# itz-sayak/C-Users-Sayakdutta-Self-Supervised-Arbitrary-Scale-Point-Cloud-Upsampling-via-SNN

Measured on AMD Instinct MI355X. Metric: upsampled query-points/sec (kNN + fn fwd + rotate + fd fwd + displace), 4x scale, M=48 T=4, higher is better.
Workload: dtype f32 (GEMMs as 3 x f16 MFMA with f32 accumulation; outer kNN f64); 1 GPU; synthetic sphere N=5000 (seed 0), B=4096 grid queries per GPU per step, M=48, T=4, fn k=[24,18,12] emb 640, fd k=32 scales [8,16,32,48] emb 768, conditioned-random weights seed 0, in-patch kNN recomputed every batch; cloud_points=5000, neighbours=48, outer_knn=f64 brute force, parallelism=query shards x1

## Files before the change

### c-users-sayakdutta-self-supervised-arbitrary-scale-point-cloud-upsampling-via-snn_amd/_lib.py

```python
import ctypes
import os
from ctypes import POINTER, c_char_p, c_double, c_float, c_int, c_int32, c_int64, c_void_p

_HERE = os.path.dirname(os.path.abspath(__file__))
LIB_PATH = os.environ.get("SAPCU_LIB_PATH") or os.path.join(_HERE, "csrc", "libsapcu_hip.so")
EXACT_LIB_PATH = os.path.join(_HERE, "csrc", "libsapcu_hip_exact.so")

FN_TAPS = ("stem", "block1", "block2", "block3", "pooled", "enc", "logits")
FD_TAPS = ("fused0", "spikes", "knn", "pooled", "enc", "x0")
KIND_FN, KIND_FD = 0, 1
ABI_VERSION = 2


class SapcuLibraryError(RuntimeError):
    """The HIP library is absent or unloadable (never silently replaced by a CPU path)."""


class SapcuError(RuntimeError):
    """A C entry point returned a non-zero status: args = (code, text)."""


_SIGNATURES = {
    "sapcu_abi_version": (c_int, []),
    "sapcu_last_error": (c_char_p, []),
# ... 43 lines not shown
    "sapcu_gemm_f32": (c_int, [c_void_p, c_int64, c_int, c_int, c_void_p, c_int, c_void_p, c_void_p, c_int, c_void_p,
                               c_int, c_void_p, c_int, c_int, c_void_p]),
    "sapcu_to_split_rows": (c_int, [c_void_p, c_int64, c_int, c_int, c_void_p, c_int, c_void_p]),
    "sapcu_posenc_gemm_f32": (c_int, [c_void_p, c_int64, c_int, c_void_p, c_void_p, c_void_p, c_int, c_void_p, c_void_p,
                                      c_int, c_int, c_void_p, c_void_p, c_void_p, c_void_p, c_int, c_void_p]),
    "sapcu_model_gemm_mode": (c_int, [c_void_p, POINTER(c_int), POINTER(c_int)]),
    "sapcu_model_fused_blocks": (c_int, [c_void_p, c_int, POINTER(c_int)]),
    "sapcu_fn_edge_chain_workspace_bytes": (c_int64, [c_int64, c_int, c_int]),
    "sapcu_fn_edge_chain_f32": (c_int, [c_void_p, c_void_p, c_int64, c_int, c_int, c_int] + [c_void_p] * 12 + [c_int, c_int, c_void_p, c_void_p,
                                        c_int64, c_void_p]),
}

EXPORTS = tuple(_SIGNATURES)

_SEEDS_SIGNATURES = {
    "sapcu_dense_seeds_workspace_bytes": (c_int64, [c_int64, c_int64]),
    "sapcu_dense_seeds_f64": (c_int, [c_void_p, c_int64, c_double, c_void_p, c_int64, c_int64, POINTER(c_int64), POINTER(c_int64),
                              c_void_p, c_int64, c_void_p]),
}
SEEDS_EXPORTS = tuple(_SEEDS_SIGNATURES)

_INTERNAL_SIGNATURES = {
    "sapcu_internal_fold_affine_host": (c_int, [c_void_p, c_void_p, c_void_p, c_void_p, c_int, c_int, c_void_p, c_void_p]),
}
_lib = None


def load(path=None):
    global _lib
    if _lib is not None and path is None:
        return _lib
    p = path or LIB_PATH
    if not os.path.exists(p):
        raise SapcuLibraryError(
            "HIP library not built: %s is missing. Run `make -C %s` (needs hipcc, gfx950). "
            "There is no CPU fallback." % (p, os.path.dirname(p)))
    try:
        lib = ctypes.CDLL(p)
    except OSError as e:
        raise SapcuLibraryError("cannot load %s: %s" % (p, e)) from e
    for name, (res, args) in list(_SIGNATURES.items()) + list(_SEEDS_SIGNATURES.items()) + list(_INTERNAL_SIGNATURES.items()):
        try:
            fn = getattr(lib, name)
        except AttributeError as e:
            raise SapcuLibraryError("%s does not export %s" % (p, name)) from e
        fn.restype = res
# ... 22 lines not shown
```

### c-users-sayakdutta-self-supervised-arbitrary-scale-point-cloud-upsampling-via-snn_amd/csrc/fd_encoder.hip

```cpp
#include <type_traits>

#include "common.h"
#include "gemm_epi.h"
#include "ops.h"

namespace sapcu {
typedef _Float16 half8 __attribute__((ext_vector_type(8)));

#ifdef FE_STAMPS
#define FE_STAMP(IDX)                                                                                                   \
    do {                                                                                                                \
        if (a.tap_spikes && threadIdx.x == 0)                                                                           \
            reinterpret_cast<unsigned long long*>(a.tap_spikes)[(int64_t)blockIdx.x * 32 + (IDX)] = __builtin_amdgcn_s_memtime(); \
    } while (0)
#else
#define FE_STAMP(IDX) do { } while (0)
#endif

constexpr int FE_M = 48;
constexpr int FE_NT = 512;
constexpr int FE_XLD = 448;
constexpr int FE_OFF_R2 = 0;
constexpr int FE_R2_BYTES = 65536;
constexpr int FE_OFF_XS = FE_R2_BYTES;
constexpr int FE_OFF_XYZ = FE_OFF_XS + FE_M * FE_XLD * 4;
constexpr int FE_OFF_IDX0 = FE_OFF_XYZ + FE_M * 16;
constexpr int FE_OFF_IDXL = FE_OFF_IDX0 + FE_M * FE_M;
constexpr int FE_OFF_XX = FE_OFF_IDXL + FE_M * FE_M;
constexpr int FE_LDS = 163840;
constexpr int FE_OFF_X3L = FE_OFF_R2 + 32768;
constexpr int FE_OFF_BEST = FE_OFF_XYZ;
static_assert(FE_OFF_BEST + 6 * 4 * 8 * 16 * 4 <= FE_LDS && FE_OFF_X3L + 16 * 512 * 4 <= FE_OFF_XYZ, "fd encoder: multi_scale_conv areas");
constexpr int FE_F_LD = 36;
constexpr int FE_KEYS_OFF = 2 * 64 * FE_F_LD * 4;
constexpr int FE_TLD = 36;
constexpr int FE_TILE = FE_M * FE_TLD;
static_assert(8 * FE_TILE * 4 <= FE_R2_BYTES, "fd encoder: staging tiles");
static_assert(FE_OFF_XX + 256 <= FE_LDS && FE_LDS <= 163840, "fd encoder: LDS budget");
static_assert(FE_KEYS_OFF + FE_M * (FE_M + 1) * 4 <= FE_R2_BYTES, "fd encoder: score keys");
// ... 107 lines not shown
#pragma unroll
                for (int i = 0; i < RC; ++i)
#pragma unroll
                    for (int j = hc * HC; j < (hc + 1) * HC && j < NCS; ++j)
                        acc[rc * RC + i][j] = __builtin_amdgcn_mfma_f32_16x16x32_f16(ah[i], wh[j], acc[rc * RC + i][j], 0, 0, 0);
            }
            __builtin_amdgcn_sched_barrier(0);
#pragma unroll
            for (int j = hc * HC; j < (hc + 1) * HC && j < NCS; ++j) {
                wh[j] = fe_wfrag(wp, nk_all, cs[j], sn, 0, lane);
                wl[j] = fe_wfrag(wp, nk_all, cs[j], sn, 1, lane);
            }
        }
    }
    if (Wh) {
#pragma unroll
        for (int j = 0; j < NCARRY; ++j) {
            (*Wh)[j] = wh[j];
            (*Wl)[j] = wl[j];
        }
    }
}

__device__ __forceinline__ int fe_wave_sum(int v) {
    v += __builtin_amdgcn_update_dpp(0, v, 0xB1, 0xF, 0xF, true);
    v += __builtin_amdgcn_update_dpp(0, v, 0x4E, 0xF, 0xF, true);
    v += __builtin_amdgcn_update_dpp(0, v, 0x141, 0xF, 0xF, true);
    v += __builtin_amdgcn_update_dpp(0, v, 0x140, 0xF, 0xF, true);
    return __builtin_amdgcn_readlane(v, 0) + __builtin_amdgcn_readlane(v, 16) + __builtin_amdgcn_readlane(v, 32) +
           __builtin_amdgcn_readlane(v, 48);
}

template <typename Fill>
__device__ __forceinline__ void fe_knn(unsigned char* R2, float* xx, unsigned char* idx_out, int m, int c, int k, Fill fill,
                                       int32_t* __restrict__ tap, int tid) {
    float* Fb = reinterpret_cast<float*>(R2);
    unsigned* K = reinterpret_cast<unsigned*>(R2 + FE_KEYS_OFF);
    const int lane = tid & 63, wave = __builtin_amdgcn_readfirstlane(tid >> 6);
    const int r16 = lane & 15, g4 = lane >> 4;
    const int bi0 = 0, bj0 = wave < 3 ? wave : 0;
    const int bi1 = wave == 1 ? 2 : 1, bj1 = wave == 2 ? 1 : 2;
    f32x4 acc0 = {0.f, 0.f, 0.f, 0.f}, acc1 = {0.f, 0.f, 0.f, 0.f};
    float myxx = 0.f;
    __syncthreads();
    if (wave >= 4) fill(Fb, 0, min(32, c), tid - 256);
    __syncthreads();
    int buf = 0;
    for (int c0 = 0; c0 < c; c0 += 32, buf ^= 1) {
        const int cw = min(32, c - c0);
        const float* F = Fb + buf * (64 * FE_F_LD);
        if (wave >= 4) {
            if (c0 + 32 < c) fill(Fb + (buf ^ 1) * (64 * FE_F_LD), c0 + 32, min(32, c - c0 - 32), tid - 256);
        } else if (wave < 3) {
            const float* fa0 = F + (16 * bi0 + r16) * FE_F_LD + g4;
            const float* fb0 = F + (16 * bj0 + r16) * FE_F_LD + g4;
            const float* fa1 = F + (16 * bi1 + r16) * FE_F_LD + g4;
            const float* fb1 = F + (16 * bj1 + r16) * FE_F_LD + g4;
            if (cw == 32) {
// ... 7 lines not shown
                }
#pragma unroll
                for (int s4 = 0; s4 < 8; ++s4) {
                    acc0 = __builtin_amdgcn_mfma_f32_16x16x4f32(a0[s4], b0[s4], acc0, 0, 0, 0);
                    acc1 = __builtin_amdgcn_mfma_f32_16x16x4f32(a1[s4], b1[s4], acc1, 0, 0, 0);
                }
            } else {
                for (int cc = 0; cc < cw; cc += 4) {
                    acc0 = __builtin_amdgcn_mfma_f32_16x16x4f32(fa0[cc], fb0[cc], acc0, 0, 0, 0);
                    acc1 = __builtin_amdgcn_mfma_f32_16x16x4f32(fa1[cc], fb1[cc], acc1, 0, 0, 0);
                }
            }
        } else if (lane < m) {
            const float* fr = F + lane * FE_F_LD;
            for (int cc2 = 0; cc2 < cw; ++cc2) {
                const float sq = __fmul_rn(fr[cc2], fr[cc2]);
                myxx = (c0 == 0 && cc2 == 0) ? sq : __fadd_rn(myxx, sq);
            }
        }
        __syncthreads();
    }
    if (wave == 3 && lane < m) xx[lane] = myxx;
    __syncthreads();
    if (wave < 3) {
#pragma unroll
        for (int q = 0; q < 2; ++q) {
            const int bi = q ? bi1 : bi0, bj = q ? bj1 : bj0;
            const f32x4 acc = q ? acc1 : acc0;
            const int j = 16 * bj + r16;
#pragma unroll
            for (int e = 0; e < 4; ++e) {
                const int i = 16 * bi + 4 * g4 + e;
                if (i < m && j < m) {
                    const float inner = __fmul_rn(-2.0f, acc[e]);
                    K[i * (m + 1) + j] = float_max_key(__fadd_rn(__fsub_rn(__fsub_rn(-xx[j], inner), xx[i]), 0.0f));
                    if (bi != bj) K[j * (m + 1) + i] = float_max_key(__fadd_rn(__fsub_rn(__fsub_rn(-xx[i], inner), xx[j]), 0.0f));
                }
            }
        }
    }
    __syncthreads();
    const int full = m * (m - 1) / 2;
    for (int i = wave; i < m; i += FE_NT / 64) {
        const unsigned key0 = lane < m ? K[i * (m + 1) + lane] : 0u;
        int r0 = 0;
        for (int jb = 0; jb < m; jb += 8) {
#pragma unroll
            for (int u = 0; u < 8; ++u) r0 += (unsigned)__builtin_amdgcn_readlane(key0, (jb + u) & 63) > key0;
        }
        const int tot = fe_wave_sum(lane < m ? r0 : 0);
        if (tot != full) {
            const unsigned long long k0 = ((unsigned long long)key0 << 32) | (unsigned)~lane;
            r0 = 0;
            for (int jb = 0; jb < m; jb += 8) {
#pragma unroll
                for (int u = 0; u < 8; ++u) {
                    const int jp = jb + u;
                    const unsigned long long kv = ((unsigned long long)(unsigned)__builtin_amdgcn_readlane(key0, jp & 63) << 32) | (unsigned)~jp;
                    r0 += kv > k0;
                }
            }
        }
        if (lane < m && r0 < k) {
            idx_out[i * FE_M + r0] = (unsigned char)lane;
            if (tap) tap[i * k + r0] = lane;
        }
    }
}

constexpr int FE_PR = 64;
constexpr int FE_TP = FE_M / 3;

__device__ __forceinline__ void fe_put_at(unsigned char* p, float v) {
    v = settle(v);
    const _Float16 hi = (_Float16)v;
    *reinterpret_cast<_Float16*>(p) = hi;
    *reinterpret_cast<_Float16*>(p + FE_PR * 64) = (_Float16)__builtin_fmaf((float)hi, -1.0f, v);
}

template <int KIND, bool FAST>
__device__ __forceinline__ void fe_emit4(const float (&x)[4], const NeuronP& p, int t0, int nemit, unsigned char* const (&pe)[4], int pt0,
                                         int m, bool count, int* __restrict__ gate, float* __restrict__ tap, int64_t tap_tstride) {
    const int total = FAST ? 4 : t0 + nemit;
    {
        NeuronStep2<KIND == 1> n0(p), n1(p);
        const f32x2 z = f32x2{0.f, 0.f};
        bool o0 = false, o1 = false;
        if (FAST) {
// ... 70 lines not shown
            if (a.tap_knn) a.tap_knn[tab_off + e] = v;
        }
    } else {
        FeNP pn = fe_load_np(a.nprm, COFF_IN + (tid & 31));
        auto fill = [&](float* F, int c0, int cw, int ftid) {
            const int cc = ftid & 31;
            const NeuronP p = fe_np(pn);
            pn = fe_load_np(a.nprm, COFF_IN + (c0 + 32 < CIN ? c0 + 32 : c0) + cc);
#pragma unroll
            for (int n = 0; n < 8; n += 2) {
                const int ia = (ftid >> 5) + 8 * n, ib = ia + 8;
                if (ia < FE_M) {
                    const f32x2 sp = fe_spike0<KIND_IN>(f32x2{XS[ia * FE_XLD + COFF_IN + c0 + cc],
                                                              XS[(ib < FE_M ? ib : ia) * FE_XLD + COFF_IN + c0 + cc]}, p);
                    F[ia * FE_F_LD + cc] = ia < m ? sp.x : 0.f;
                    F[ib * FE_F_LD + cc] = (ib < m && ib < FE_M) ? sp.y : 0.f;
                } else {
                    F[ia * FE_F_LD + cc] = 0.f;
                    F[ib * FE_F_LD + cc] = 0.f;
                }
            }
            (void)cw;
        };
        fe_knn(R2, xx, IDXL, m, CIN, kk, fill, a.tap_knn ? a.tap_knn + tab_off : nullptr, tid);
    }
    __syncthreads();
    FE_STAMP(4 * L);
    {
        const int cc = tid & 63;
        FeNP pn2 = fe_load_np(a.nprm, COFF_IN + cc);
        for (int c0 = 0; c0 < CIN; c0 += 64) {
            const NeuronP p = fe_np(pn2);
            pn2 = fe_load_np(a.nprm, COFF_IN + (c0 + 64 < CIN ? c0 + 64 : c0) + cc);
#pragma unroll
            for (int n = 0; n < 6; n += 2) {
                const int ia = (tid >> 6) + 8 * n, ib = ia + 8;
                const f32x2 sp = fe_spike0<KIND_IN>(f32x2{XS[ia * FE_XLD + COFF_IN + c0 + cc], XS[ib * FE_XLD + COFF_IN + c0 + cc]}, p);
                fe_put<64>(R2, ia, c0 + cc, sp.x);
                fe_put<64>(R2, ib, c0 + cc, sp.y);
#ifdef FE_DEBUG_PANEL
                if (a.tap_x0 && ia < m) a.tap_x0[((a.s0 + patch_i) * m + ia) * 960 + COFF_IN + c0 + cc] = sp.x;
                if (a.tap_x0 && ib < m) a.tap_x0[((a.s0 + patch_i) * m + ib) * 960 + COFF_IN + c0 + cc] = sp.y;
#endif
            }
        }
    }
    __syncthreads();
    FE_STAMP(4 * L + 1);
    const bool active = L != 1 || w < 4;
    f32x4 acc[NPW][3][4];
    if (active) {
#pragma unroll
        for (int q = 0; q < NPW; ++q) {
            const int pr = w + 8 * q;
            const int css[4] = {2 * pr, 2 * pr + 1, 2 * (COUT / 32 + pr), 2 * (COUT / 32 + pr) + 1};
            fe_gemm16<4, 3>(R2, 4096, reinterpret_cast<const half8*>(a.edge_wp[L - 1]), CIN / 32, css, lane, acc[q]);
        }
    }
    __syncthreads();
    FE_STAMP(4 * L + 2);
    float* SAw = reinterpret_cast<float*>(R2) + w * FE_TILE;
    const int c16 = lane & 15, g4 = lane >> 4;
    const int qd = lane & 7, g6 = 6 * (lane >> 3);
#pragma unroll
    for (int q = 0; q < NPW; ++q) {
        float pre[3][2][4];
        if (active) {
            const int col0 = 32 * (w + 8 * q) + c16;
            const float sh[2] = {a.shift[L - 1][col0], a.shift[L - 1][col0 + 16]};
#pragma unroll
            for (int rs = 0; rs < 3; ++rs)
#pragma unroll
                for (int cj = 0; cj < 2; ++cj)
#pragma unroll
                    for (int e = 0; e < 4; ++e)
                        SAw[(16 * rs + 4 * g4 + e) * FE_TLD + 16 * cj + c16] = __fadd_rn(__fmul_rn(acc[q][rs][cj][e], 0.0625f), 0.0f);
            asm volatile("s_waitcnt lgkmcnt(0)" ::: "memory");
            __builtin_amdgcn_wave_barrier();
            {
                float4 mx[6];
#pragma unroll
                for (int r = 0; r < 6; ++r) mx[r] = make_float4(-__builtin_huge_valf(), -__builtin_huge_valf(), -__builtin_huge_valf(), -__builtin_huge_valf());
                const unsigned char* ir0 = IDXL + g6 * FE_M;
                const float* tq = SAw + 4 * qd;
                int j = 0;
                for (; j + 4 <= kk; j += 4) {
                    unsigned pk[6];
#pragma unroll
                    for (int r = 0; r < 6; ++r) pk[r] = *reinterpret_cast<const unsigned*>(ir0 + r * FE_M + j);
#pragma unroll
                    for (int r = 0; r < 6; ++r) {
                        const float4 v0 = *reinterpret_cast<const float4*>(tq + (pk[r] & 255u) * FE_TLD);
                        const float4 v1 = *reinterpret_cast<const float4*>(tq + ((pk[r] >> 8) & 255u) * FE_TLD);
                        const float4 v2 = *reinterpret_cast<const float4*>(tq + ((pk[r] >> 16) & 255u) * FE_TLD);
                        const float4 v3 = *reinterpret_cast<const float4*>(tq + (pk[r] >> 24) * FE_TLD);
                        mx[r].x = fmaxf(fmaxf(mx[r].x, v0.x), fmaxf(v1.x, fmaxf(v2.x, v3.x)));
                        mx[r].y = fmaxf(fmaxf(mx[r].y, v0.y), fmaxf(v1.y, fmaxf(v2.y, v3.y)));
                        mx[r].z = fmaxf(fmaxf(mx[r].z, v0.z), fmaxf(v1.z, fmaxf(v2.z, v3.z)));
                        mx[r].w = fmaxf(fmaxf(mx[r].w, v0.w), fmaxf(v1.w, fmaxf(v2.w, v3.w)));
                    }
                }
                for (; j < kk; ++j) {
#pragma unroll
                    for (int r = 0; r < 6; ++r) {
                        const float4 v0 = *reinterpret_cast<const float4*>(tq + ir0[r * FE_M + j] * FE_TLD);
                        mx[r].x = fmaxf(mx[r].x, v0.x);
                        mx[r].y = fmaxf(mx[r].y, v0.y);
                        mx[r].z = fmaxf(mx[r].z, v0.z);
                        mx[r].w = fmaxf(mx[r].w, v0.w);
                    }
                }
                asm volatile("s_waitcnt lgkmcnt(0)" ::: "memory");
                __builtin_amdgcn_wave_barrier();
#pragma unroll
                for (int r = 0; r < 6; ++r) *reinterpret_cast<float4*>(SAw + (g6 + r) * FE_TLD + 4 * qd) = mx[r];
                asm volatile("s_waitcnt lgkmcnt(0)" ::: "memory");
                __builtin_amdgcn_wave_barrier();
            }
#pragma unroll
            for (int rs = 0; rs < 3; ++rs)
#pragma unroll
                for (int cj = 0; cj < 2; ++cj)
#pragma unroll
                    for (int e = 0; e < 4; ++e) {
                        const int row = 16 * rs + 4 * g4 + e;
                        const float mxv = SAw[row * FE_TLD + 16 * cj + c16];
                        const float xb = __fadd_rn(__fmul_rn(acc[q][rs][2 + cj][e], 0.0625f), 0.0f);
                        pre[rs][cj][e] = lrelu02(__fadd_rn(__fsub_rn(mxv, xb), sh[cj]));
                        if (a.tap_x0 && row < m) a.tap_x0[((a.s0 + patch_i) * m + row) * 960 + COFF_OUT + col0 + 16 * cj] = pre[rs][cj][e];
                    }
            asm volatile("s_waitcnt lgkmcnt(0)" ::: "memory");
            __builtin_amdgcn_wave_barrier();
            if (L <= 2) {
#pragma unroll
                for (int rs = 0; rs < 3; ++rs)
#pragma unroll
                    for (int cj = 0; cj < 2; ++cj)
#pragma unroll
                        for (int e = 0; e < 4; ++e) XS[(16 * rs + 4 * g4 + e) * FE_XLD + COFF_OUT + col0 + 16 * cj] = pre[rs][cj][e];
            } else {
#pragma unroll
                for (int rs = 0; rs < 3; ++rs)
#pragma unroll
                    for (int cj = 0; cj < 2; ++cj)
#pragma unroll
                        for (int e = 0; e < 4; ++e) SAw[(16 * rs + 4 * g4 + e) * FE_TLD + 16 * cj + c16] = pre[rs][cj][e];
            }
        }
        if (L == 3) {
            __syncthreads();
            const float* SA = reinterpret_cast<const float*>(R2);
#pragma unroll
            for (int jj = 0; jj < 2; ++jj) {
                const int c3l = 2 * jj + 1 - (w & 1);
#pragma unroll
                for (int th = 0; th < 3; ++th)
#pragma unroll
                    for (int e = 0; e < 4; ++e)
                        x3[th][2 * q + jj][e] = SA[(2 * c3l + (lane >> 5)) * FE_TILE + (FE_TP * th + 4 * (w >> 1) + e) * FE_TLD + (lane & 31)];
            }
            __syncthreads();
        }
    }
    __syncthreads();
    FE_STAMP(4 * L + 3);
}

template <bool GENERAL>
__global__ __launch_bounds__(FE_NT, 1) void fd_encoder_kernel(const FdEncArgs a) {
    extern __shared__ __attribute__((aligned(1024))) unsigned char smem[];
    float* XS = reinterpret_cast<float*>(smem + FE_OFF_XS);
    unsigned char* R2 = smem + FE_OFF_R2;
    float4* XYZ = reinterpret_cast<float4*>(smem + FE_OFF_XYZ);
    unsigned char* IDX0 = smem + FE_OFF_IDX0;
    float* xx = reinterpret_cast<float*>(smem + FE_OFF_XX);
    const int tid = threadIdx.x;
    const int lane = tid & 63, w = __builtin_amdgcn_readfirstlane(tid >> 6);
    const int m = a.m;
    const int64_t patch_i = blockIdx.x;
    const float* __restrict__ pp = a.patch + patch_i * m * 3;

    for (int e = tid; e < FE_M; e += FE_NT)
        XYZ[e] = e < m ? make_float4(pp[3 * e], pp[3 * e + 1], pp[3 * e + 2], 0.f) : make_float4(0.f, 0.f, 0.f, 0.f);
    for (int e = tid; e < 2 * FE_M * FE_M / 4; e += FE_NT) reinterpret_cast<unsigned*>(IDX0)[e] = 0u;
    __syncthreads();
    FE_STAMP(0);
    {
        auto fill = [&](float* F, int c0, int cw, int ftid) {
            {
                const int i = ftid >> 2, cc = ftid & 3;
                const float v = reinterpret_cast<const float*>(XYZ)[4 * (i < FE_M ? i : 0) + cc];
                F[i * FE_F_LD + cc] = i < m ? v : 0.f;
            }
            (void)c0; (void)cw;
        };
        fe_knn(R2, xx, IDX0, m, 3, a.kmax0, fill, nullptr, tid);
    }
    __syncthreads();
    FE_STAMP(1);
    {
        const float* XYZf = reinterpret_cast<const float*>(XYZ);
        const int r16 = lane & 15, g4 = lane >> 4;
        float wb[4][4][2], bb[4];
#pragma unroll
        for (int sc = 0; sc < 4; ++sc) {
#pragma unroll
            for (int ct = 0; ct < 4; ++ct)
#pragma unroll
                for (int kstep = 0; kstep < 2; ++kstep) {
                    const int k = 4 * kstep + g4;
                    wb[sc][ct][kstep] = (sc < a.nscale && k < 6) ? a.e0_w[((int64_t)sc * 64 + 16 * ct + r16) * 6 + k] : 0.f;
                }
            bb[sc] = sc < a.nscale ? a.e0_b[sc * 64 + lane] : 0.f;
        }
        int ksv[4];
#pragma unroll
        for (int sc = 0; sc < 4; ++sc) ksv[sc] = sc < a.nscale ? a.ks[sc] : 0;
        float big = 0.f;
        for (int i = w; i < m; i += FE_NT / 64) {
// ... 174 lines not shown
                FE_TACC(fe_t_epi);
            };
            third(std::integral_constant<int, 0>{});
            third(std::integral_constant<int, 1>{});
            third(std::integral_constant<int, 2>{});
            if (cbw < ncb) {
                int lane_e = lane;
                asm volatile("" : "+v"(lane_e));
                const float* bl = BESTL;
                asm volatile("" : "+v"(bl));
                const int tt = lane_e >> 4, r16e = lane_e & 15;
#pragma unroll
                for (int j = 0; j < 6; ++j) {
                    const float bias = a.msc_b[16 * css[j] + r16e];
                    const float raw = bl[512 * j];
                    if (tt < nemit)
                        a.pooled[((int64_t)(t0 + tt) * a.b + patch_i) * a.emb + 16 * css[j] + r16e] = lrelu02(__fadd_rn(__fmul_rn(raw, 0.0625f), bias));
                }
            }
        }
    }
#ifdef FE_STAMPS
    if (a.tap_spikes && threadIdx.x == 0) {
        unsigned long long* st = reinterpret_cast<unsigned long long*>(a.tap_spikes) + (int64_t)blockIdx.x * 32;
        st[17] = fe_t_emit;
        st[18] = fe_t_mfma;
        st[28] = fe_t_start;
        st[29] = fe_t_epi;
        st[19] = __builtin_amdgcn_s_memtime();
    }
#endif
}

constexpr int FM_OFF_BEST = 32768;
constexpr int FM_LDS = FM_OFF_BEST + 6 * 4 * 8 * 16 * 4;

template <bool GENERAL>
__global__ __launch_bounds__(FE_NT, 1) void fd_msc_kernel(const FdMscArgs a) {
    extern __shared__ __attribute__((aligned(1024))) unsigned char smem[];
    unsigned char* R2 = smem;
    const int tid = threadIdx.x;
    const int lane = tid & 63, w = __builtin_amdgcn_readfirstlane(tid >> 6);
    const int m = a.m;
    const int64_t patch_i = blockIdx.x;
    const float* __restrict__ xp = a.x0 + patch_i * m * 960;
    const int cw = w & 1, rg = w >> 1;
    const int nsweep = a.emb / 768 + (a.emb % 768 ? 1 : 0);
// ... 178 lines not shown
```

### c-users-sayakdutta-self-supervised-arbitrary-scale-point-cloud-upsampling-via-snn_amd/csrc/model.hip

```cpp
#include <stdarg.h>
#include <stdlib.h>

#include <new>
#include <vector>

#include "common.h"
#include "ops.h"

namespace sapcu {

static thread_local char g_err[512] = "";

void set_error(const char* fmt, ...) {
    va_list ap;
    va_start(ap, fmt);
    vsnprintf(g_err, sizeof(g_err), fmt, ap);
    va_end(ap);
}

enum FnSlot {
    FN_STEM_W = 0, FN_STEM_B, FN_STEM_LIF,
    FN_BLK0 = 3,
    FN_FINAL_W = FN_BLK0 + 63, FN_FINAL_B, FN_FINAL_LIF,
    FN_FCOUT_W, FN_FCOUT_B,
// ... 976 lines not shown
        if (m->w16_hi) (void)hipFree(m->w16_hi);
        if (m->w16_lo) (void)hipFree(m->w16_lo);
        if (m->chain_w) (void)hipFree(m->chain_w);
        if (m->ovf_dev) (void)hipFree(m->ovf_dev);
        if (m->blob) (void)hipFree(m->blob);
        if (m->ks_dev) (void)hipFree(m->ks_dev);
        if (m->gate_dev) (void)hipFree(m->gate_dev);
        if (m->fde_w) (void)hipFree(m->fde_w);
        if (m->fde_nprm) (void)hipFree(m->fde_nprm);
        delete m;
        return rc;
    }
    *out = m;
    return SAPCU_OK;
}

int sapcu_internal_fold_affine_host(const float* w_out, const float* b_out, const float* w_fc2, const float* b_fc2, int d, int n,
                                    float* w_fold_out, float* b_fold_out) {
    SAPCU_CHECK_ARG(w_out && b_out && w_fc2 && b_fc2 && w_fold_out && b_fold_out && d >= 1 && n >= 1, "fold_affine: bad argument");
    fold_affine_f64(w_out, b_out, w_fc2, b_fc2, d, n, w_fold_out, b_fold_out);
    return SAPCU_OK;
}

int sapcu_model_destroy(sapcu_model_t m) {
    if (!m) return SAPCU_OK;
    if (m->w16_hi) (void)hipFree(m->w16_hi);
    if (m->w16_lo) (void)hipFree(m->w16_lo);
    if (m->chain_w) (void)hipFree(m->chain_w);
    if (m->ovf_dev) (void)hipFree(m->ovf_dev);
    if (m->blob) (void)hipFree(m->blob);
    if (m->ks_dev) (void)hipFree(m->ks_dev);
    if (m->gate_dev) (void)hipFree(m->gate_dev);
    if (m->fde_w) (void)hipFree(m->fde_w);
    if (m->fde_nprm) (void)hipFree(m->fde_nprm);
    delete m;
    return SAPCU_OK;
}

int64_t sapcu_workspace_bytes(sapcu_model_t m, int64_t b, int m_pts) {
    if (!m || b < 0 || m_pts < 1 || m_pts > 128) {
        set_error("workspace_bytes: bad argument");
        return SAPCU_ERR_ARG;
    }
    return m->kind == SAPCU_KIND_FN ? fn_ws_bytes(m, b, m_pts) : fd_ws_bytes(m, b, m_pts);
}

// ... 48 lines not shown
```

### c-users-sayakdutta-self-supervised-arbitrary-scale-point-cloud-upsampling-via-snn_amd/csrc/ops.h

```cpp
#pragma once
#include "common.h"

namespace sapcu {

int launch_patch_knn_strided(const float* feat, int64_t b, int64_t pstride, int m, int c, int ld, int k,
                             int32_t* idx, hipStream_t st);
int launch_patch_knn_multi(const float* feat, int64_t b, int64_t pstride, int m, int c, int ld, int ntab,
                           const int* ks, int32_t* const* idx, hipStream_t st);
int launch_patch_knn(const float* feat, int64_t b, int m, int c, int ld, int k, int32_t* idx, hipStream_t st);
int launch_neuron_selfloop(const float* x, int64_t rows, int ch, int T, const float* md, const float* ta,
                           const float* rd, const float* tb, const float* dT, const float* rh, float* so, float* mo,
                           float* to, float* ro, hipStream_t st);
int launch_neuron_drive(const float* x, int64_t rows, int ch, int T, const float* md, const float* ta, const float* rd, const float* tb,
                        const float* dT, const float* rh, int pairv, float* so, float* mo, float* to, float* ro, int* gate, hipStream_t st);
int launch_fn_stem(const float* patch, int64_t rows, const float* w, const float* bias, const float* lif, int T,
                   float* out, hipStream_t st);
int launch_fn_pe1(const float* patch, const int32_t* idx, int64_t rows, int m, int kk, int d, const float* w,
                  const float* bias, const float* lif, int T, float* out, int split, hipStream_t st);
struct ChainArgs {
    int64_t P;
    int m;
    const int2* tab;
    const float4* pd;
    const float* qkv;
    int ldq;
    const float* wd;
    const float* bd;
    const float* lifd;
    const _Float16* w1p;
    const float* b1;
    const float* lif1;
    const _Float16* w2p;
// ... 82 lines not shown
```

### c-users-sayakdutta-self-supervised-arbitrary-scale-point-cloud-upsampling-via-snn_amd/csrc/patch_ops.hip

```cpp
#include "common.h"
#include "ops.h"
#include "gemm_epi.h"

namespace sapcu {

constexpr int PK_CH = 32;

struct KnnOut {
    int32_t* idx[3];
    int k[3];
    int n;
};

constexpr int PK_LD = 36;

template <int NT>
__global__ __launch_bounds__(NT) void patch_knn_kernel(const float* __restrict__ feat, int64_t pstride, int m,
                                                       int c, int ld, const KnnOut out) {
    extern __shared__ float sm[];
    unsigned* K = reinterpret_cast<unsigned*>(sm);
    float* xx = sm + m * (m + 1);
    float* F = xx + m;
    const int tid = threadIdx.x;
    const int lane = tid & 63, wave = __builtin_amdgcn_readfirstlane(tid >> 6);
    const int r16 = lane & 15, g4 = lane >> 4;
    const float* base = feat + (int64_t)blockIdx.x * pstride;
    const int nb = (m + 15) >> 4, mpad = 16 * nb;
    constexpr int NW = NT / 64;
    constexpr int NBW = NT == 256 ? 3 : 5;
    int bi[NBW], bj[NBW];
    {
        int t = 0, q = 0;
#pragma unroll
        for (int u = 0; u < NBW; ++u) bi[u] = bj[u] = -1;
        for (int i = 0; i < nb; ++i)
            for (int j = i; j < nb; ++j, ++t)
                if (t % NW == wave) {
#pragma unroll
                    for (int u = 0; u < NBW; ++u)
// ... 32 lines not shown
            for (int cc = 0; cc < cw; ++cc) {
                const float sq = __fmul_rn(fr[cc], fr[cc]);
                myxx = (c0 == 0 && cc == 0) ? sq : __fadd_rn(myxx, sq);
            }
        }
    }
    if (tid < m) xx[tid] = myxx;
    __syncthreads();
#pragma unroll
    for (int u = 0; u < NBW; ++u) {
        if (bi[u] < 0) continue;
        const int j = 16 * bj[u] + r16;
#pragma unroll
        for (int e = 0; e < 4; ++e) {
            const int i = 16 * bi[u] + 4 * g4 + e;
            if (i < m && j < m) {
                const float inner = __fmul_rn(-2.0f, acc[u][e]);
                K[i * (m + 1) + j] = float_max_key(__fadd_rn(__fsub_rn(__fsub_rn(-xx[j], inner), xx[i]), 0.0f));
                if (bi[u] != bj[u]) K[j * (m + 1) + i] = float_max_key(__fadd_rn(__fsub_rn(__fsub_rn(-xx[i], inner), xx[j]), 0.0f));
            }
        }
    }
    __syncthreads();
    const int full = m * (m - 1) / 2;
    for (int i = wave; i < m; i += NT / 64) {
        const unsigned* row = K + i * (m + 1);
        const int j0 = lane, j1 = lane + 64;
        const unsigned key0 = j0 < m ? row[j0] : 0u, key1 = j1 < m ? row[j1] : 0u;
        int r0 = 0, r1 = 0;
        if (m <= 64) {
            for (int jb = 0; jb < m; jb += 8) {
#pragma unroll
                for (int u = 0; u < 8; ++u) r0 += (unsigned)__builtin_amdgcn_readlane(key0, jb + u) > key0;
            }
        } else {
            for (int jb = 0; jb < 64; jb += 8) {
#pragma unroll
                for (int u = 0; u < 8; ++u) {
                    const unsigned kv = (unsigned)__builtin_amdgcn_readlane(key0, jb + u);
                    r0 += kv > key0;
                    r1 += kv > key1;
                }
            }
            for (int jb = 64; jb < m; jb += 8) {
#pragma unroll
                for (int u = 0; u < 8; ++u) {
// ... 25 lines not shown
        }
        for (int t = 0; t < out.n; ++t) {
            const int k = out.k[t];
            int32_t* o = out.idx[t] + ((int64_t)blockIdx.x * m + i) * k;
            if (j0 < m && r0 < k) o[r0] = j0;
            if (j1 < m && r1 < k) o[r1] = j1;
        }
    }
}

int launch_patch_knn_multi(const float* feat, int64_t b, int64_t pstride, int m, int c, int ld, int ntab,
                           const int* ks, int32_t* const* idx, hipStream_t st) {
    if (b == 0) return SAPCU_OK;
    SAPCU_CHECK_ARG(m >= 1 && m <= 128 && c >= 1 && ntab >= 1 && ntab <= 3, "patch_knn: need 1<=m<=128, 1..3 tables (m=%d)", m);
    KnnOut out;
    out.n = ntab;
    for (int t = 0; t < 3; ++t) {
        out.idx[t] = t < ntab ? idx[t] : nullptr;
        out.k[t] = t < ntab ? ks[t] : 0;
        if (t < ntab) SAPCU_CHECK_ARG(ks[t] >= 1 && ks[t] <= m && idx[t], "patch_knn: need 1<=k<=m (k=%d m=%d)", ks[t], m);
    }
    const int nb = (m + 15) / 16;
    const size_t lds = (size_t)(m * (m + 1) + m + 16 * nb * PK_LD) * sizeof(float);
#define SAPCU_PK(NT)                                                                                                  \
    do {                                                                                                              \
        static DeviceOnce once;                                                                                       \
        if (lds > 65536) SAPCU_SET_MAX_LDS(once, (&patch_knn_kernel<NT>), 98304);                                      \
        hipLaunchKernelGGL((patch_knn_kernel<NT>), dim3((unsigned)b), dim3(NT), lds, st, feat, pstride, m, c, ld, out); \
    } while (0)
    if (m <= 64) SAPCU_PK(256);
    else SAPCU_PK(512);
#undef SAPCU_PK
    SAPCU_CHECK_LAUNCH();
    return SAPCU_OK;
}

int launch_patch_knn_strided(const float* feat, int64_t b, int64_t pstride, int m, int c, int ld, int k,
                             int32_t* idx, hipStream_t st) {
    return launch_patch_knn_multi(feat, b, pstride, m, c, ld, 1, &k, &idx, st);
}

int launch_patch_knn(const float* feat, int64_t b, int m, int c, int ld, int k, int32_t* idx, hipStream_t st) {
    return launch_patch_knn_strided(feat, b, (int64_t)m * ld, m, c, ld, k, idx, st);
}

template <bool EIF, bool PAIRV>
__global__ __launch_bounds__(256) void neuron_drive_kernel(const float* __restrict__ x, int64_t rows, int ch, int T, const float* md,
                                                           const float* ta, const float* rd, const float* tb, const float* dT,
                                                           const float* rh, float* __restrict__ so, float* mo, float* to, float* ro,
                                                           int* __restrict__ gate) {
    const int64_t t = (int64_t)blockIdx.x * blockDim.x + threadIdx.x;
    const int64_t npair = PAIRV ? rows * ((ch + 1) / 2) : ((rows + 1) / 2) * ch;
    if (t >= npair) return;
    int64_t ea, eb;
    int ca, cb;
// ... 934 lines not shown
```

### profiles/fd_stamps.py

```python
#!/usr/bin/env python3
import os
import sys
import time

import numpy as np
import torch

ROOT = os.path.dirname(os.path.dirname(os.path.abspath(__file__)))
sys.path.insert(0, ROOT)
import bench


def main():
    dev = torch.device("cuda", 0)
    from sapcu_amd import testing as T, generation as gen
    B, M = 4096, 48
    os.environ["SAPCU_FD_FUSED"] = "1"
    _, fd, _, _ = bench.build_models(dev)
    cloud = torch.as_tensor(T.sphere_cloud(5000, 0), device=dev)
    seeds = torch.as_tensor(T.grid_queries(B, 0), device=dev)
    _, _, patch = gen.knn_gather(cloud, seeds, M)
    stamps = torch.zeros((B, 32), dtype=torch.int64, device=dev)
    buf = stamps.view(torch.float32)
    with torch.no_grad():
        fd(patch)
        torch.cuda.synchronize()
        t0 = time.perf_counter()
        fd(patch, taps={"spikes": buf})
        torch.cuda.synchronize()
        wall = time.perf_counter() - t0
    s = stamps.cpu().numpy().astype(np.float64)
    total = s[:, 19] - s[:, 0]
    names = {1: "xyz kNN", 2: "block-0 EdgeConv", 3: "scale fusion GEMM",
             4: "L1 kNN", 5: "L1 panel", 6: "L1 GEMM", 7: "L1 max",
             8: "L2 kNN", 9: "L2 panel", 10: "L2 GEMM", 11: "L2 max",
             12: "L3 kNN", 13: "L3 panel", 14: "L3 GEMM", 15: "L3 max + transposition", 16: "(to MSC start)"}
    print("forward wall %.2f ms; per patch (median over %d patches), s_memtime ticks:" % (wall * 1e3, B))
    print("  total %.0f ticks" % np.median(total))
    prev = 0
    for i in range(1, 17):
        d = s[:, i] - s[:, prev]
        print("  %-26s %8.0f  (%.1f %%)" % (names[i], np.median(d), 100 * np.median(d) / np.median(total)))
        prev = i
    msc = s[:, 19] - s[:, 16]
    print("  %-26s %8.0f  (%.1f %%)  = emission %.0f + MFMA rounds %.0f + epilogues etc. %.0f" % (
        "multi_scale_conv", np.median(msc), 100 * np.median(msc) / np.median(total), np.median(s[:, 17]), np.median(s[:, 18]),
        np.median(msc - s[:, 17] - s[:, 18])))
    if s[:, 28].any() or s[:, 29].any():
        print("  multi_scale_conv, per patch: starts of the thirds (x0 dump, accumulators, first fragments) %.0f, epilogues of the thirds %.0f"
              % (np.median(s[:, 28]), np.median(s[:, 29])))
    if s[:, 20].any():
        for base, name in ((20, "xyz search"), (24, "L3 search")):
            print("  %s: to end of chunk loop %.0f, keys %.0f" % (name, np.median(s[:, base + 1] - s[:, base]), np.median(s[:, base + 2] - s[:, base + 1])))
        print("  xyz rank + tail %.0f ; L3 rank + tail %.0f" % (np.median(s[:, 1] - s[:, 22]), np.median(s[:, 12] - s[:, 26])))
    print("  => %.3f us per tick if the forward is %d patches per CU back to back" % (wall * 1e6 / (B / 256.0) / np.median(total), B // 256))


if __name__ == "__main__":
    main()
```

Measured before the change: 126,600 query-points/s.

## Replace per-row rank counting in patch kNN with a 64-lane bitonic sorting network

The in-patch kNN used an O(m) per-lane readlane rank count, plus a fallback pass to break ties. It is replaced by a wave-wide bitonic sort of 64-bit (key, ~lane) pairs using DPP and permlane swaps, processing three rows per wave at once in both the fused FD encoder and the standalone patch_knn kernel. This removes the serial readlane loops and the tie fallback at the cost of a fixed set of sort stages and more registers. Stamp instrumentation and a test entry point are added; the old scan path stays reachable through an environment variable.

```diff
diff --git a/c-users-sayakdutta-self-supervised-arbitrary-scale-point-cloud-upsampling-via-snn_amd/_lib.py b/c-users-sayakdutta-self-supervised-arbitrary-scale-point-cloud-upsampling-via-snn_amd/_lib.py
--- a/c-users-sayakdutta-self-supervised-arbitrary-scale-point-cloud-upsampling-via-snn_amd/_lib.py
+++ b/c-users-sayakdutta-self-supervised-arbitrary-scale-point-cloud-upsampling-via-snn_amd/_lib.py
@@ -89,6 +89,7 @@
 
 _INTERNAL_SIGNATURES = {
     "sapcu_internal_fold_affine_host": (c_int, [c_void_p, c_void_p, c_void_p, c_void_p, c_int, c_int, c_void_p, c_void_p]),
+    "sapcu_internal_rank_net64": (c_int, [c_void_p, c_int64, c_void_p, c_void_p]),
 }
 _lib = None
 
diff --git a/c-users-sayakdutta-self-supervised-arbitrary-scale-point-cloud-upsampling-via-snn_amd/csrc/fd_encoder.hip b/c-users-sayakdutta-self-supervised-arbitrary-scale-point-cloud-upsampling-via-snn_amd/csrc/fd_encoder.hip
--- a/c-users-sayakdutta-self-supervised-arbitrary-scale-point-cloud-upsampling-via-snn_amd/csrc/fd_encoder.hip
+++ b/c-users-sayakdutta-self-supervised-arbitrary-scale-point-cloud-upsampling-via-snn_amd/csrc/fd_encoder.hip
@@ -3,18 +3,27 @@
 #include "common.h"
 #include "gemm_epi.h"
 #include "ops.h"
+#include "rank_net.h"
 
 namespace sapcu {
 typedef _Float16 half8 __attribute__((ext_vector_type(8)));
 
 #ifdef FE_STAMPS
+#define FE_STAMP_BASE(A) ((A).tap_spikes ? reinterpret_cast<unsigned long long*>((A).tap_spikes) + (int64_t)blockIdx.x * 64 : nullptr)
 #define FE_STAMP(IDX)                                                                                                   \
     do {                                                                                                                \
-        if (a.tap_spikes && threadIdx.x == 0)                                                                           \
-            reinterpret_cast<unsigned long long*>(a.tap_spikes)[(int64_t)blockIdx.x * 32 + (IDX)] = __builtin_amdgcn_s_memtime(); \
+        if (a.tap_spikes && threadIdx.x == 0) FE_STAMP_BASE(a)[IDX] = __builtin_amdgcn_s_memtime();                      \
     } while (0)
+#define FE_STAMP_P(P, IDX)                                                                                              \
+    do {                                                                                                                \
+        if ((P) && threadIdx.x == 0) (P)[IDX] = __builtin_amdgcn_s_memtime();                                           \
+    } while (0)
+#define FE_TICK(V) V = __builtin_amdgcn_s_memtime()
 #else
+#define FE_STAMP_BASE(A) static_cast<unsigned long long*>(nullptr)
 #define FE_STAMP(IDX) do { } while (0)
+#define FE_STAMP_P(P, IDX) do { } while (0)
+#define FE_TICK(V) do { } while (0)
 #endif
 
 constexpr int FE_M = 48;
@@ -168,18 +177,9 @@
     }
 }
 
-__device__ __forceinline__ int fe_wave_sum(int v) {
-    v += __builtin_amdgcn_update_dpp(0, v, 0xB1, 0xF, 0xF, true);
-    v += __builtin_amdgcn_update_dpp(0, v, 0x4E, 0xF, 0xF, true);
-    v += __builtin_amdgcn_update_dpp(0, v, 0x141, 0xF, 0xF, true);
-    v += __builtin_amdgcn_update_dpp(0, v, 0x140, 0xF, 0xF, true);
-    return __builtin_amdgcn_readlane(v, 0) + __builtin_amdgcn_readlane(v, 16) + __builtin_amdgcn_readlane(v, 32) +
-           __builtin_amdgcn_readlane(v, 48);
-}
-
 template <typename Fill>
 __device__ __forceinline__ void fe_knn(unsigned char* R2, float* xx, unsigned char* idx_out, int m, int c, int k, Fill fill,
-                                       int32_t* __restrict__ tap, int tid) {
+                                       int32_t* __restrict__ tap, int tid, unsigned long long* stamps = nullptr) {
     float* Fb = reinterpret_cast<float*>(R2);
     unsigned* K = reinterpret_cast<unsigned*>(R2 + FE_KEYS_OFF);
     const int lane = tid & 63, wave = __builtin_amdgcn_readfirstlane(tid >> 6);
@@ -233,6 +233,7 @@
     }
     if (wave == 3 && lane < m) xx[lane] = myxx;
     __syncthreads();
+    FE_STAMP_P(stamps, 0);
     if (wave < 3) {
 #pragma unroll
         for (int q = 0; q < 2; ++q) {
@@ -251,30 +252,23 @@
         }
     }
     __syncthreads();
-    const int full = m * (m - 1) / 2;
-    for (int i = wave; i < m; i += FE_NT / 64) {
-        const unsigned key0 = lane < m ? K[i * (m + 1) + lane] : 0u;
-        int r0 = 0;
-        for (int jb = 0; jb < m; jb += 8) {
-#pragma unroll
-            for (int u = 0; u < 8; ++u) r0 += (unsigned)__builtin_amdgcn_readlane(key0, (jb + u) & 63) > key0;
-        }
-        const int tot = fe_wave_sum(lane < m ? r0 : 0);
-        if (tot != full) {
-            const unsigned long long k0 = ((unsigned long long)key0 << 32) | (unsigned)~lane;
-            r0 = 0;
-            for (int jb = 0; jb < m; jb += 8) {
-#pragma unroll
-                for (int u = 0; u < 8; ++u) {
-                    const int jp = jb + u;
-                    const unsigned long long kv = ((unsigned long long)(unsigned)__builtin_amdgcn_readlane(key0, jp & 63) << 32) | (unsigned)~jp;
-                    r0 += kv > k0;
-                }
-            }
-        }
-        if (lane < m && r0 < k) {
-            idx_out[i * FE_M + r0] = (unsigned char)lane;
-            if (tap) tap[i * k + r0] = lane;
+    FE_STAMP_P(stamps, 1);
+    for (int i0 = wave; i0 < m; i0 += 3 * (FE_NT / 64)) {
+        unsigned key[3];
+        int nbr[3];
+#pragma unroll
+        for (int r = 0; r < 3; ++r) {
+            const int i = i0 + r * (FE_NT / 64);
+            key[r] = (lane < m && i < m) ? K[i * (m + 1) + lane] : 0u;
+        }
+        rank_net64<3>(key, nbr, lane);
+#pragma unroll
+        for (int r = 0; r < 3; ++r) {
+            const int i = i0 + r * (FE_NT / 64);
+            if (i < m && lane < k) {
+                idx_out[i * FE_M + lane] = (unsigned char)nbr[r];
+                if (tap) tap[i * k + lane] = nbr[r];
+            }
         }
     }
 }
@@ -391,7 +385,8 @@
             }
             (void)cw;
         };
-        fe_knn(R2, xx, IDXL, m, CIN, kk, fill, a.tap_knn ? a.tap_knn + tab_off : nullptr, tid);
+        fe_knn(R2, xx, IDXL, m, CIN, kk, fill, a.tap_knn ? a.tap_knn + tab_off : nullptr, tid,
+               FE_STAMP_BASE(a) ? FE_STAMP_BASE(a) + 32 + 4 * L : nullptr);
     }
     __syncthreads();
     FE_STAMP(4 * L);
@@ -431,12 +426,16 @@
     float* SAw = reinterpret_cast<float*>(R2) + w * FE_TILE;
     const int c16 = lane & 15, g4 = lane >> 4;
     const int qd = lane & 7, g6 = 6 * (lane >> 3);
+#ifdef FE_STAMPS
+    unsigned long long tk0 = 0, tk1 = 0, tk2 = 0, tk3 = 0, tk_stage = 0, tk_max = 0, tk_pick = 0;
+#endif
 #pragma unroll
     for (int q = 0; q < NPW; ++q) {
         float pre[3][2][4];
         if (active) {
             const int col0 = 32 * (w + 8 * q) + c16;
             const float sh[2] = {a.shift[L - 1][col0], a.shift[L - 1][col0 + 16]};
+            FE_TICK(tk0);
 #pragma unroll
             for (int rs = 0; rs < 3; ++rs)
 #pragma unroll
@@ -446,6 +445,7 @@
                         SAw[(16 * rs + 4 * g4 + e) * FE_TLD + 16 * cj + c16] = __fadd_rn(__fmul_rn(acc[q][rs][cj][e], 0.0625f), 0.0f);
             asm volatile("s_waitcnt lgkmcnt(0)" ::: "memory");
             __builtin_amdgcn_wave_barrier();
+            FE_TICK(tk1);
             {
                 float4 mx[6];
 #pragma unroll
@@ -486,6 +486,7 @@
                 asm volatile("s_waitcnt lgkmcnt(0)" ::: "memory");
                 __builtin_amdgcn_wave_barrier();
             }
+            FE_TICK(tk2);
 #pragma unroll
             for (int rs = 0; rs < 3; ++rs)
 #pragma unroll
@@ -500,6 +501,12 @@
                     }
             asm volatile("s_waitcnt lgkmcnt(0)" ::: "memory");
             __builtin_amdgcn_wave_barrier();
+#ifdef FE_STAMPS
+            FE_TICK(tk3);
+            tk_stage += tk1 - tk0;
+            tk_max += tk2 - tk1;
+            tk_pick += tk3 - tk2;
+#endif
             if (L <= 2) {
 #pragma unroll
                 for (int rs = 0; rs < 3; ++rs)
@@ -533,6 +540,13 @@
     }
     __syncthreads();
     FE_STAMP(4 * L + 3);
+#ifdef FE_STAMPS
+    if (a.tap_spikes && threadIdx.x == 0) {
+        FE_STAMP_BASE(a)[48 + 4 * (L - 1)] = tk_stage;
+        FE_STAMP_BASE(a)[48 + 4 * (L - 1) + 1] = tk_max;
+        FE_STAMP_BASE(a)[48 + 4 * (L - 1) + 2] = tk_pick;
+    }
+#endif
 }
 
 template <bool GENERAL>
@@ -563,7 +577,7 @@
             }
             (void)c0; (void)cw;
         };
-        fe_knn(R2, xx, IDX0, m, 3, a.kmax0, fill, nullptr, tid);
+        fe_knn(R2, xx, IDX0, m, 3, a.kmax0, fill, nullptr, tid, FE_STAMP_BASE(a) ? FE_STAMP_BASE(a) + 32 : nullptr);
     }
     __syncthreads();
     FE_STAMP(1);
@@ -784,7 +798,7 @@
     }
 #ifdef FE_STAMPS
     if (a.tap_spikes && threadIdx.x == 0) {
-        unsigned long long* st = reinterpret_cast<unsigned long long*>(a.tap_spikes) + (int64_t)blockIdx.x * 32;
+        unsigned long long* st = FE_STAMP_BASE(a);
         st[17] = fe_t_emit;
         st[18] = fe_t_mfma;
         st[28] = fe_t_start;
diff --git a/c-users-sayakdutta-self-supervised-arbitrary-scale-point-cloud-upsampling-via-snn_amd/csrc/model.hip b/c-users-sayakdutta-self-supervised-arbitrary-scale-point-cloud-upsampling-via-snn_amd/csrc/model.hip
--- a/c-users-sayakdutta-self-supervised-arbitrary-scale-point-cloud-upsampling-via-snn_amd/csrc/model.hip
+++ b/c-users-sayakdutta-self-supervised-arbitrary-scale-point-cloud-upsampling-via-snn_amd/csrc/model.hip
@@ -1022,6 +1022,11 @@
     return SAPCU_OK;
 }
 
+int sapcu_internal_rank_net64(const uint32_t* keys, int64_t rows, int32_t* idx_out, void* stream) {
+    SAPCU_CHECK_ARG(keys && idx_out && rows >= 0, "rank_net64: bad argument");
+    return launch_rank_net64(keys, rows, idx_out, (hipStream_t)stream);
+}
+
 int sapcu_model_destroy(sapcu_model_t m) {
     if (!m) return SAPCU_OK;
     if (m->w16_hi) (void)hipFree(m->w16_hi);
diff --git a/c-users-sayakdutta-self-supervised-arbitrary-scale-point-cloud-upsampling-via-snn_amd/csrc/ops.h b/c-users-sayakdutta-self-supervised-arbitrary-scale-point-cloud-upsampling-via-snn_amd/csrc/ops.h
--- a/c-users-sayakdutta-self-supervised-arbitrary-scale-point-cloud-upsampling-via-snn_amd/csrc/ops.h
+++ b/c-users-sayakdutta-self-supervised-arbitrary-scale-point-cloud-upsampling-via-snn_amd/csrc/ops.h
@@ -8,6 +8,7 @@
 int launch_patch_knn_multi(const float* feat, int64_t b, int64_t pstride, int m, int c, int ld, int ntab,
                            const int* ks, int32_t* const* idx, hipStream_t st);
 int launch_patch_knn(const float* feat, int64_t b, int m, int c, int ld, int k, int32_t* idx, hipStream_t st);
+int launch_rank_net64(const unsigned* keys, int64_t rows, int32_t* idx, hipStream_t st);
 int launch_neuron_selfloop(const float* x, int64_t rows, int ch, int T, const float* md, const float* ta,
                            const float* rd, const float* tb, const float* dT, const float* rh, float* so, float* mo,
                            float* to, float* ro, hipStream_t st);
diff --git a/c-users-sayakdutta-self-supervised-arbitrary-scale-point-cloud-upsampling-via-snn_amd/csrc/patch_ops.hip b/c-users-sayakdutta-self-supervised-arbitrary-scale-point-cloud-upsampling-via-snn_amd/csrc/patch_ops.hip
--- a/c-users-sayakdutta-self-supervised-arbitrary-scale-point-cloud-upsampling-via-snn_amd/csrc/patch_ops.hip
+++ b/c-users-sayakdutta-self-supervised-arbitrary-scale-point-cloud-upsampling-via-snn_amd/csrc/patch_ops.hip
@@ -1,6 +1,10 @@
 #include "common.h"
 #include "ops.h"
 #include "gemm_epi.h"
+#include "rank_net.h"
+
+#include <cstdlib>
+#include <cstring>
 
 namespace sapcu {
 
@@ -14,7 +18,7 @@
 
 constexpr int PK_LD = 36;
 
-template <int NT>
+template <int NT, bool NET>
 __global__ __launch_bounds__(NT) void patch_knn_kernel(const float* __restrict__ feat, int64_t pstride, int m,
                                                        int c, int ld, const KnnOut out) {
     extern __shared__ float sm[];
@@ -93,6 +97,28 @@
         }
     }
     __syncthreads();
+    if (NET) {
+        for (int i0 = wave; i0 < m; i0 += 3 * NW) {
+            unsigned key[3];
+            int nbr[3];
+#pragma unroll
+            for (int r = 0; r < 3; ++r) {
+                const int i = i0 + r * NW;
+                key[r] = (lane < m && i < m) ? K[i * (m + 1) + lane] : 0u;
+            }
+            rank_net64<3>(key, nbr, lane);
+#pragma unroll
+            for (int r = 0; r < 3; ++r) {
+                const int i = i0 + r * NW;
+                if (i >= m) continue;
+                for (int t = 0; t < out.n; ++t) {
+                    const int k = out.k[t];
+                    if (lane < k) out.idx[t][((int64_t)blockIdx.x * m + i) * k + lane] = nbr[r];
+                }
+            }
+        }
+        return;
+    }
     const int full = m * (m - 1) / 2;
     for (int i = wave; i < m; i += NT / 64) {
         const unsigned* row = K + i * (m + 1);
@@ -164,15 +190,38 @@
     }
     const int nb = (m + 15) / 16;
     const size_t lds = (size_t)(m * (m + 1) + m + 16 * nb * PK_LD) * sizeof(float);
-#define SAPCU_PK(NT)                                                                                                  \
-    do {                                                                                                              \
-        static DeviceOnce once;                                                                                       \
-        if (lds > 65536) SAPCU_SET_MAX_LDS(once, (&patch_knn_kernel<NT>), 98304);                                      \
-        hipLaunchKernelGGL((patch_knn_kernel<NT>), dim3((unsigned)b), dim3(NT), lds, st, feat, pstride, m, c, ld, out); \
+#define SAPCU_PK(NT, NET)                                                                                                  \
+    do {                                                                                                                   \
+        static DeviceOnce once;                                                                                            \
+        if (lds > 65536) SAPCU_SET_MAX_LDS(once, (&patch_knn_kernel<NT, NET>), 98304);                                      \
+        hipLaunchKernelGGL((patch_knn_kernel<NT, NET>), dim3((unsigned)b), dim3(NT), lds, st, feat, pstride, m, c, ld, out); \
     } while (0)
-    if (m <= 64) SAPCU_PK(256);
-    else SAPCU_PK(512);
+    static const bool rank_scan = [] {
+        const char* e = getenv("SAPCU_RANK");
+        return e && !strcmp(e, "scan");
+    }();
+    if (m > 64) SAPCU_PK(512, false);
+    else if (rank_scan) SAPCU_PK(256, false);
+    else SAPCU_PK(256, true);
 #undef SAPCU_PK
+    SAPCU_CHECK_LAUNCH();
+    return SAPCU_OK;
+}
+
+__global__ __launch_bounds__(256) void rank_net64_kernel(const unsigned* __restrict__ keys, int64_t rows, int32_t* __restrict__ idx) {
+    const int lane = threadIdx.x & 63;
+    const int64_t row = (int64_t)blockIdx.x * 4 + (threadIdx.x >> 6);
+    if (row >= rows) return;
+    const unsigned key[1] = {keys[row * 64 + lane]};
+    int nbr[1];
+    rank_net64<1>(key, nbr, lane);
+    idx[row * 64 + lane] = nbr[0];
+}
+
+int launch_rank_net64(const unsigned* keys, int64_t rows, int32_t* idx, hipStream_t st) {
+    if (rows == 0) return SAPCU_OK;
+    SAPCU_CHECK_ARG(rows > 0 && rows < (1LL << 31), "rank_net64: bad row count");
+    hipLaunchKernelGGL(rank_net64_kernel, dim3((unsigned)((rows + 3) / 4)), dim3(256), 0, st, keys, rows, idx);
     SAPCU_CHECK_LAUNCH();
     return SAPCU_OK;
 }
diff --git a/c-users-sayakdutta-self-supervised-arbitrary-scale-point-cloud-upsampling-via-snn_amd/csrc/rank_net.h b/c-users-sayakdutta-self-supervised-arbitrary-scale-point-cloud-upsampling-via-snn_amd/csrc/rank_net.h
--- /dev/null
+++ b/c-users-sayakdutta-self-supervised-arbitrary-scale-point-cloud-upsampling-via-snn_amd/csrc/rank_net.h
@@ -0,0 +1,65 @@
+#pragma once
+#include "common.h"
+
+namespace sapcu {
+
+template <int J>
+__device__ __forceinline__ unsigned rn_xor_dpp(unsigned x) {
+    static_assert(J == 1 || J == 2 || J == 4 || J == 8, "rank network: DPP partner distances");
+    if (J == 1) return (unsigned)__builtin_amdgcn_update_dpp((int)x, (int)x, 0xB1, 0xF, 0xF, false);
+    if (J == 2) return (unsigned)__builtin_amdgcn_update_dpp((int)x, (int)x, 0x4E, 0xF, 0xF, false);
+    if (J == 8) return (unsigned)__builtin_amdgcn_update_dpp((int)x, (int)x, 0x128, 0xF, 0xF, false);
+    const int t = __builtin_amdgcn_update_dpp((int)x, (int)x, 0x104, 0xF, 0x5, false);
+    return (unsigned)__builtin_amdgcn_update_dpp(t, (int)x, 0x114, 0xF, 0xA, false);
+}
+
+template <int K, int J, int R>
+__device__ __forceinline__ void rn_stage(unsigned (&hi)[R], unsigned (&lo)[R], int lane) {
+    const bool keep_max = ((lane & J) == 0) == ((lane & K) == 0);
+#pragma unroll
+    for (int r = 0; r < R; ++r) {
+        if constexpr (J < 16) {
+            const unsigned ohi = rn_xor_dpp<J>(hi[r]), olo = rn_xor_dpp<J>(lo[r]);
+            const bool other_gt = (((unsigned long long)ohi << 32) | olo) > (((unsigned long long)hi[r] << 32) | lo[r]);
+            const bool take = other_gt == keep_max;
+            hi[r] = take ? ohi : hi[r];
+            lo[r] = take ? olo : lo[r];
+        } else {
+            const auto ph = J == 16 ? __builtin_amdgcn_permlane16_swap(hi[r], hi[r], false, false)
+                                    : __builtin_amdgcn_permlane32_swap(hi[r], hi[r], false, false);
+            const auto pl = J == 16 ? __builtin_amdgcn_permlane16_swap(lo[r], lo[r], false, false)
+                                    : __builtin_amdgcn_permlane32_swap(lo[r], lo[r], false, false);
+            const bool a_gt = (((unsigned long long)ph[0] << 32) | pl[0]) > (((unsigned long long)ph[1] << 32) | pl[1]);
+            const bool want_max = (lane & K) == 0;
+            const bool take_a = a_gt == (((lane & J) == 0) == want_max);
+            hi[r] = take_a ? ph[0] : ph[1];
+            lo[r] = take_a ? pl[0] : pl[1];
+        }
+    }
+}
+
+template <int K, int J, int R>
+__device__ __forceinline__ void rn_merge(unsigned (&hi)[R], unsigned (&lo)[R], int lane) {
+    rn_stage<K, J, R>(hi, lo, lane);
+    if constexpr (J > 1) rn_merge<K, J / 2, R>(hi, lo, lane);
+}
+
+template <int R>
+__device__ __forceinline__ void rank_net64(const unsigned (&key)[R], int (&index)[R], int lane) {
+    unsigned hi[R], lo[R];
+#pragma unroll
+    for (int r = 0; r < R; ++r) {
+        hi[r] = key[r];
+        lo[r] = ~(unsigned)lane;
+    }
+    rn_merge<2, 1, R>(hi, lo, lane);
+    rn_merge<4, 2, R>(hi, lo, lane);
+    rn_merge<8, 4, R>(hi, lo, lane);
+    rn_merge<16, 8, R>(hi, lo, lane);
+    rn_merge<32, 16, R>(hi, lo, lane);
+    rn_merge<64, 32, R>(hi, lo, lane);
+#pragma unroll
+    for (int r = 0; r < R; ++r) index[r] = (int)~lo[r];
+}
+
+}
diff --git a/profiles/fd_stamps.py b/profiles/fd_stamps.py
--- a/profiles/fd_stamps.py
+++ b/profiles/fd_stamps.py
@@ -20,7 +20,7 @@
     cloud = torch.as_tensor(T.sphere_cloud(5000, 0), device=dev)
     seeds = torch.as_tensor(T.grid_queries(B, 0), device=dev)
     _, _, patch = gen.knn_gather(cloud, seeds, M)
-    stamps = torch.zeros((B, 32), dtype=torch.int64, device=dev)
+    stamps = torch.zeros((B, 64), dtype=torch.int64, device=dev)
     buf = stamps.view(torch.float32)
     with torch.no_grad():
         fd(patch)
@@ -49,10 +49,15 @@
     if s[:, 28].any() or s[:, 29].any():
         print("  multi_scale_conv, per patch: starts of the thirds (x0 dump, accumulators, first fragments) %.0f, epilogues of the thirds %.0f"
               % (np.median(s[:, 28]), np.median(s[:, 29])))
-    if s[:, 20].any():
-        for base, name in ((20, "xyz search"), (24, "L3 search")):
-            print("  %s: to end of chunk loop %.0f, keys %.0f" % (name, np.median(s[:, base + 1] - s[:, base]), np.median(s[:, base + 2] - s[:, base + 1])))
-        print("  xyz rank + tail %.0f ; L3 rank + tail %.0f" % (np.median(s[:, 1] - s[:, 22]), np.median(s[:, 12] - s[:, 26])))
+    print("  neighbour searches:          scores       keys       rank")
+    for sidx, (first, last, name) in enumerate(((0, 1, "xyz"), (3, 4, "L1"), (7, 8, "L2"), (11, 12, "L3"))):
+        b0 = 32 + 4 * sidx
+        sc, ky, rk = s[:, b0] - s[:, first], s[:, b0 + 1] - s[:, b0], s[:, last] - s[:, b0 + 1]
+        print("    %-22s %10.0f %10.0f %10.0f" % (name, np.median(sc), np.median(ky), np.median(rk)))
+    print("  neighbour maxima (wave 0):    stage        max    pick-up")
+    for L in (1, 2, 3):
+        b0 = 48 + 4 * (L - 1)
+        print("    %-22s %10.0f %10.0f %10.0f" % ("L%d" % L, np.median(s[:, b0]), np.median(s[:, b0 + 1]), np.median(s[:, b0 + 2])))
     print("  => %.3f us per tick if the forward is %d patches per CU back to back" % (wall * 1e6 / (B / 256.0) / np.median(total), B // 256))
 
 
```

Result: no change. 127,600 query-points/s, median of 6 (+0.8%).
